# kchmck/p25rx

Measured on AMD Instinct MI355X. Metric: IQ Msamples/s through FM-demod+C4FM slice, higher is better.
Workload: dtype f32

## Files before the change

### p25rx_amd/csrc/p25fe_api.hip

```cpp
#include "p25fe_kernels.hip"

#include <hip/hip_ext.h>
#include <math.h>
#include <stdio.h>
#include <stdlib.h>
#include <string.h>

#include <algorithm>
#include <array>
#include <chrono>
#include <new>
#include <utility>
#include <string>
#include <vector>

#include "p25fe_jit.h"

using namespace p25k;

namespace {

constexpr size_t BBPAD = 256;
constexpr size_t SHARD_HALO = 2560;
static_assert(SHARD_HALO >= (size_t)(DEC * (PLPAD + CLK_L + 160) + TMAX) && 160 >= TMAX + TMAX - 1 && SHARD_HALO % 8 == 0, "shard halo");
// ... 221 lines not shown
    }
    void k1_events(bool ext_events, hipEvent_t* e0, hipEvent_t* e1)
    {
        *e0 = *e1 = nullptr;
        if (slot < 0 || !ext_events) return;
        *e0 = ev[(size_t)slot * 5 + 0]; *e1 = ev[(size_t)slot * 5 + 1];
        mask[(size_t)slot] |= 3u;
    }
};

constexpr size_t WIN_PARITY = 2, WIN_RING = 4;
struct WinSlot {
    hipEvent_t h2d_begin = nullptr, h2d_end = nullptr;
    hipEvent_t comp_begin = nullptr, comp_end = nullptr;
    hipEvent_t on_host = nullptr;
    std::array<hipEvent_t*, 5> all() { return {&h2d_begin, &h2d_end, &comp_begin, &comp_end, &on_host}; }
};
struct Windows {
    DevBuf buf[WIN_PARITY], dib[WIN_PARITY], res, anc;
    PinBuf stage[WIN_PARITY], out;
    hipStream_t cs = nullptr, os = nullptr;
    WinSlot slot[WIN_RING];
    WinSlot& of(size_t k) { return slot[k % WIN_RING]; }
    hipError_t ensure()
    {
        if (cs) return hipSuccess;
        hipError_t e = hipStreamCreateWithFlags(&cs, hipStreamNonBlocking);
        if (e == hipSuccess) e = hipStreamCreateWithFlags(&os, hipStreamNonBlocking);
        for (WinSlot& s : slot) for (hipEvent_t* x : s.all()) if (e == hipSuccess) e = hipEventCreate(x);
        return e;
    }
};

}

struct p25fe {
    p25fe_config_t cfg;
    int C = 1, n_cu = 256;
    Taps taps;
    int k1_p = 5;
    int variant = P25FE_VARIANT_BUILTIN;
    bool dflt = true;
    bool long_taps = false;
    int phase = P25FE_DECIM_PHASE;
    int n_avg = BOX;
    bool u8_lut_mode = false;
    float u8_scale = 0.0f, u8_offset = 0.0f;
    int track = 0;
    bool causal_ok = false;
    long look = 0;
    bool ext_events = true;
    int rx_cus = 0;
    int run_depth = 2;
    int sh_depth = MAX_LANES;

    int last_hip = 0;
    DevBuf d_taps;
    hipModule_t jit_mod = nullptr;
    hipFunction_t jit_fn[2][3] = {{nullptr, nullptr, nullptr}, {nullptr, nullptr, nullptr}};
    hipStream_t stream = nullptr, rx_stream = nullptr;
    const long* rs_idx = nullptr; size_t rs_n = 0, rs_stride = 0;
    Lane lanes[MAX_LANES];
    int cur = 0, lane_q[MAX_LANES - 1] = {1, 2, 3};
    int pl_lane = -1; size_t pl_blocks = 0;
    Lane& lane() { return lanes[cur]; }
    RxScratch& rx() { return lanes[cur].s; }
    const RxScratch& rx() const { return lanes[cur].s; }
    DevBuf power_partial, chunk_cnt, evrec, evnext, evoff;
    unsigned long long ev_seq = 0;
    PinBuf hin, hbb, hout;
    unsigned chunk_seq = 0;
    Windows win; StreamState state; Prof prof; ShardCtx sh;
};

struct PlanarGeo {
    size_t n_tiles, n_blocks;
    explicit PlanarGeo(size_t n_bb)
    {
        n_tiles = (n_bb + TS - 1) / TS;
        if (n_tiles == 0) n_tiles = 1;
        n_blocks = (size_t)TWORDS * n_tiles + 6;
    }
    size_t floats() const { return n_blocks * PL_BLK; }
    size_t words() const { return n_blocks * SPS; }
};

constexpr size_t MAX_RANGE_BB = (size_t)0x7ff00000u * 10u;
static inline bool position_refused(uint64_t pos) { return pos >= P25FE_MAX_POSITION; }

struct Resolved {
    Taps taps;
    bool long_taps;
    bool lut_affine;
    float u8_scale, u8_offset;
    bool dflt;
};

static inline bool finite_f(float v) { return v - v == 0.0f; }
static inline bool same_bits(float a, float b) { return memcmp(&a, &b, sizeof a) == 0; }

static bool lut_is_affine(const float* lut, float sc, float of)
{
    for (int b = 0; b < 256; ++b)
        if (!same_bits(lut[b], fmaf((float)b, sc, of))) return false;
    return true;
}
// ... 260 lines not shown
    try {
        h->state.reset((size_t)h->C);
    } catch (...) {
        return P25FE_ERR_NOMEM;
    }
    return P25FE_OK;
}

int p25fe_create(const p25fe_config_t* cfg, p25fe_t** out)
{
    if (!cfg || !out) return P25FE_ERR_ARG;
    *out = nullptr;
    if (cfg->abi_version != P25FE_ABI_VERSION || cfg->n_channels < 1 || cfg->n_channels > 65535 ) return P25FE_ERR_ARG;
    Resolved rs;
    if (int rrc = resolve_config(cfg, &rs)) return rrc;
    int ndev = 0;
    if (hipGetDeviceCount(&ndev) != hipSuccess || ndev <= 0 || cfg->device < 0 || cfg->device >= ndev)
        return P25FE_ERR_NO_DEVICE;
    if (hipSetDevice(cfg->device) != hipSuccess) return P25FE_ERR_NO_DEVICE;
    hipDeviceProp_t prop;
    if (hipGetDeviceProperties(&prop, cfg->device) != hipSuccess) return P25FE_ERR_NO_DEVICE;
    if (strncmp(prop.gcnArchName, "gfx950", 6) != 0) return P25FE_ERR_NO_DEVICE;

    p25fe_t* h = new (std::nothrow) p25fe;
    if (!h) return P25FE_ERR_NOMEM;
    h->cfg = *cfg;
    h->C = cfg->n_channels;
    h->track = cfg->symbol_clock & 0xff;
    h->causal_ok = (cfg->symbol_clock & P25FE_CLOCK_CAUSAL_OK) != 0;
    h->look = h->track ? CLK_L : 0;
    h->n_cu = prop.multiProcessorCount > 0 ? prop.multiProcessorCount : 256;
    h->taps = rs.taps;
    h->phase = cfg->decim_phase;
    h->n_avg = rs.taps.n_avg;
    h->long_taps = rs.long_taps;
    h->u8_lut_mode = !rs.lut_affine;
    h->u8_scale = rs.u8_scale; h->u8_offset = rs.u8_offset;
    h->variant = rs.dflt ? P25FE_VARIANT_BUILTIN : P25FE_VARIANT_GENERIC;
    h->dflt = rs.dflt;
    if (hipStreamCreateWithFlags(&h->stream, hipStreamNonBlocking) != hipSuccess) { p25fe_destroy(h); return P25FE_ERR_HIP; }
    hipError_t e = hipSuccess;
    {
        const char* pv = getenv("P25FE_K1_P");
        h->k1_p = (pv && atoi(pv) == 3) ? 3 : 5;
        const char* ee = getenv("P25FE_EXT_EVENTS");
        h->ext_events = !(ee && atoi(ee) == 0);
        const char* rc_ = getenv("P25FE_RX_CUS");
        h->rx_cus = rc_ ? atoi(rc_) : 0;
        const char* pd = getenv("P25FE_SHARD_PIPE_DEPTH");
        if (pd && atoi(pd) >= 2 && atoi(pd) <= MAX_LANES) h->sh_depth = atoi(pd);
        if (cfg->symbol_clock != P25FE_CLOCK_FIXED) h->run_depth = 3;
        const char* rd = getenv("P25FE_PIPE_DEPTH");
        if (rd && atoi(rd) >= 2 && atoi(rd) <= MAX_LANES) h->run_depth = atoi(rd);
    }
    if (e == hipSuccess) e = h->d_taps.ensure(sizeof(Taps));
    if (e == hipSuccess) e = hipMemcpy(h->d_taps.p, &h->taps, sizeof(Taps), hipMemcpyHostToDevice);
    if (e != hipSuccess) { p25fe_destroy(h); return P25FE_ERR_HIP; }
    {
        std::vector<char> code;
        std::string path;
        bool from_cache = false;
        int var = choose_variant(cfg, rs, &code, &path, &from_cache);
        if (var < 0) { p25fe_destroy(h); return var; }
        if (var == P25FE_VARIANT_SPECIALIZED) {
            bool ok = false;
            try {
                hipError_t me = hipModuleLoadData(&h->jit_mod, code.data());
                if (me != hipSuccess && from_cache) {
                    (void)hipGetLastError();
                    t_jit_log += "cached code object " + path + " did not load: recompiling\n";
                    const std::string store = p25jit::default_cache_dir();
                    if (path.compare(0, store.size() + 1, store + "/") == 0) (void)remove(path.c_str());
                    h->jit_mod = nullptr;
                    if (p25jit::get_code(jit_spec(rs), {}, true, store, false, code, path, t_jit_log)) me = hipModuleLoadData(&h->jit_mod, code.data());
                }
                ok = me == hipSuccess;
                for (int f = 0; f < 2 && ok; ++f)
                    for (int k = 0; k < 3 && ok; ++k)
                        ok = hipModuleGetFunction(&h->jit_fn[f][k], h->jit_mod, p25jit::KERNEL_NAMES[f][k]) == hipSuccess;
                if (!ok) { (void)hipGetLastError(); t_jit_log += "loading the specialised code object failed\n"; }
            } catch (...) {
                ok = false;
            }
            if (!ok) {
                if (h->jit_mod) { (void)hipModuleUnload(h->jit_mod); h->jit_mod = nullptr; }
                if (cfg->specialize >= P25FE_SPECIALIZE_REQUIRE) { p25fe_destroy(h); return P25FE_ERR_JIT; }
                var = rs.dflt ? P25FE_VARIANT_BUILTIN : P25FE_VARIANT_GENERIC;
                if (var == P25FE_VARIANT_GENERIC) fallback_notice();
            }
        }
        h->variant = var;
    }
    int rc = p25fe_reset(h);
    if (rc != P25FE_OK) { p25fe_destroy(h); return rc; }
    *out = h;
    return P25FE_OK;
}

void p25fe_destroy(p25fe_t* h)
{
    if (!h) return;
    (void)hipSetDevice(h->cfg.device);
    for (hipStream_t st : {h->stream, h->rx_stream, h->win.cs, h->win.os})
        if (st) { (void)hipStreamSynchronize(st); (void)hipStreamDestroy(st); }
    if (h->jit_mod) (void)hipModuleUnload(h->jit_mod);
    for (WinSlot& s : h->win.slot) for (hipEvent_t* e : s.all()) if (*e) (void)hipEventDestroy(*e);
    for (Lane& l : h->lanes)
        for (hipEvent_t e : {l.ev_k1, l.ev_rx}) if (e) (void)hipEventDestroy(e);
    for (auto& e : h->prof.ev) if (e) (void)hipEventDestroy(e);
    delete h;
}

}

enum K1Part { K1_ALL = 0, K1_MAIN = 1, K1_HEAD = 2 };
static int format_unusable(const p25fe_t* h, int fmt)
{
    const int v = format_variant_of(h->variant, h->dflt, h->cfg.specialize, fmt);
    return v < 0 ? v : P25FE_OK;
}
struct K1Launch {
    const void* src = nullptr;
    int fmt = P25FE_FMT_CF32;
    size_t ch_stride = 0, n_hist = 0, n = 0;
    uint64_t abs0 = 0;
    float* bb = nullptr; size_t bb_stride = 0;
    float* power_dbm = nullptr;
    bool planar = false;
    K1Part part = K1_ALL;
    hipEvent_t ev0 = nullptr, ev1 = nullptr;
    const ChunkRecvArgs* chunk = nullptr;
    long* head_end = nullptr;
    unsigned* done_flag = nullptr; unsigned done_seq = 0u;
    hipStream_t stream = nullptr;
};

struct K1Plan {
    bool empty;
    K1Args a;
    int fmt, variant; bool ct; int pk;
    long n_seg;
    long head_end;
    size_t lds;
};
static int k1_plan(const p25fe_t* h, const K1Launch& L, K1Plan* p)
{
    const int fmt = L.fmt;
    const int variant = format_variant_of(h->variant, h->dflt, h->cfg.specialize, fmt);
    if (variant < 0) return variant;
    if ((reinterpret_cast<uintptr_t>(L.src) & 15u) != 0) return P25FE_ERR_ARG;
    if (h->C > 1 && (L.ch_stride % fmt_stride_unit(fmt)) != 0) return P25FE_ERR_ARG;
    if (L.chunk && (!L.planar || L.part)) return P25FE_ERR_ARG;
    const bool pro = seg_prologue(fmt);
    const long m_begin = !L.planar ? 0 : (pro ? -(long)PLPAD - h->look : -(long)HIST_BB - h->look);
    const size_t n_out = p25fe_n_baseband_h(h, L.abs0, L.n);
    const long total = (long)n_out - m_begin;
    K1Args& a = p->a;
    a.m_begin = m_begin; a.n_out = (long)n_out; p->head_end = 0;
    p->empty = total <= 0;
    if (p->empty) return P25FE_OK;
    const int pk = (L.planar || h->long_taps || variant == P25FE_VARIANT_SPECIALIZED) ? 5 : h->k1_p;
    const int t1 = h->long_taps ? TMAX : T1;
    static const long subs_env = [] { const char* e = getenv("P25FE_SUBS"); return e ? atol(e) : 0L; }();
    long subs = subs_env > 0 ? subs_env : (fmt == P25FE_FMT_U8 ? 9 : (fmt == P25FE_FMT_S16 ? P25FE_K1_SUBS_S16 : 3));
    if (L.chunk) subs = 1;
    if (subs > 32768) subs = 32768;
    const bool ct = variant != P25FE_VARIANT_GENERIC;
    const int t2e = h->long_taps ? TMAX : T2;
    const int t3geo = ct ? h->n_avg : TMAX;
    SegGeo g{pro, WV * pk, (int)subs, seg_halo_for(h->n_avg, t2e), 0, m_begin, (long)n_out};
    const int nd = g.front(t3geo, t2e);
    const long o0 = (long)(((uint64_t)h->phase + 5 - L.abs0 % 5) % 5);
    if (L.part && subs > 1 && !L.chunk) g.set_lead(nd, o0, t1);
    const long n_seg = g.count(total);
    const long pl_shift = PLPAD + h->look;
    if (L.planar && !g.planar_ok(pl_shift)) return P25FE_ERR_ARG;
    if (L.planar && n_out > MAX_RANGE_BB) return P25FE_ERR_ARG;
    long seg_first = 0, seg_count = n_seg;
    if (L.part) {
        if (L.power_dbm) return P25FE_ERR_ARG;
        const long k_min = g.head_count(n_seg, nd, o0, t1);
        if (L.part == K1_MAIN) { seg_first = k_min; seg_count = n_seg - k_min; }
        else seg_count = k_min;
        p->head_end = g.start(k_min) - m_begin;
        p->empty = seg_count <= 0;
        if (p->empty) return P25FE_OK;
    }
    if (seg_count * (long)h->C > 0x7fffffffL) return P25FE_ERR_ARG;
    p->fmt = fmt; p->variant = variant; p->ct = ct; p->pk = pk; p->n_seg = n_seg;
    a.x = L.src; a.ch_stride = (long)L.ch_stride; a.n_hist = (long)L.n_hist; a.n_new = (long)L.n; a.o0 = (int)o0; a.n_ch = h->C;
    a.bb = L.bb; a.bb_stride = (long)L.bb_stride; a.power_partial = nullptr;
    a.subs_per_seg = g.subs_per_seg; a.seg_first = (int)seg_first; a.seg_count = (int)seg_count; a.lead_segs = g.lead_segs; a.seg_halo = g.segh;
    a.bbp = nullptr; a.bbp_ch_stride = 0; a.bits = nullptr; a.bits_ch_stride = 0; a.pl_shift = (int)pl_shift;
    a.done_flag = L.planar ? L.done_flag : nullptr; a.done_seq = L.done_seq;
    if (L.planar) {
        const PlanarGeo g(n_out);
        a.bbp = h->rx().pl_f.get(); a.bbp_ch_stride = (long)g.floats();
        a.bits = reinterpret_cast<uint8_t*>(h->rx().pl_bits.get()); a.bits_ch_stride = (long)(4 * g.words());
    }
    const bool lut = fmt == P25FE_FMT_U8 && (!ct || h->u8_lut_mode);
    p->lds = h->long_taps ? k1_lds_bytes<Geo<5, 1>>(ct, lut, t3geo) : (pk == 3 ? k1_lds_bytes<Geo<3>>(ct, lut, t3geo) : k1_lds_bytes<Geo<5>>(ct, lut, t3geo));
    static const size_t lds_pad_env = [] { const char* e = getenv("P25FE_K1_LDS_PAD"); return e ? (size_t)atol(e) : (size_t)0; }();
    p->lds += lds_pad_env;
    return P25FE_OK;
}

using K1Kernel = void (*)(K1Args, const Taps*);
using ChunkKernel = void (*)(K1Args, const Taps*, ChunkTail);
template <int FMT> static K1Kernel k1_kernel_of(bool ct, int pk, bool planar, bool long_taps)
{
    if (long_taps) return planar ? k_frontend<FMT, false, 5, OUT_PLANAR, 1> : k_frontend<FMT, false, 5, OUT_LINEAR, 1>;
    if (planar) return ct ? k_frontend<FMT, true, 5, OUT_PLANAR, 0> : k_frontend<FMT, false, 5, OUT_PLANAR, 0>;
    if (pk == 3) return ct ? k_frontend<FMT, true, 3, OUT_LINEAR, 0> : k_frontend<FMT, false, 3, OUT_LINEAR, 0>;
    return ct ? k_frontend<FMT, true, 5, OUT_LINEAR, 0> : k_frontend<FMT, false, 5, OUT_LINEAR, 0>;
}
template <int FMT> static ChunkKernel chunk_kernel_of(bool ct, bool long_taps)
{
    if (long_taps) return k_chunk<FMT, false, 1>;
    return ct ? k_chunk<FMT, true, 0> : k_chunk<FMT, false, 0>;
}
static K1Kernel k1_kernel_of(int fmt, bool ct, int pk, bool planar, bool long_taps)
{
    switch (fmt) {
    case P25FE_FMT_U8: return k1_kernel_of<P25FE_FMT_U8>(ct, pk, planar, long_taps);
    case P25FE_FMT_S16: return k1_kernel_of<P25FE_FMT_S16>(ct, pk, planar, long_taps);
    default: return k1_kernel_of<P25FE_FMT_CF32>(ct, pk, planar, long_taps);
    }
}
static ChunkKernel chunk_kernel_of(int fmt, bool ct, bool long_taps)
{
    switch (fmt) {
    case P25FE_FMT_U8: return chunk_kernel_of<P25FE_FMT_U8>(ct, long_taps);
    case P25FE_FMT_S16: return chunk_kernel_of<P25FE_FMT_S16>(ct, long_taps);
    default: return chunk_kernel_of<P25FE_FMT_CF32>(ct, long_taps);
    }
}

static int launch_k1(p25fe_t* h, const K1Launch& L)
{
    K1Plan p;
    if (int rc = k1_plan(h, L, &p)) return rc;
    if (L.head_end) *L.head_end = p.head_end;
    hipStream_t st = L.stream;
    if (p.empty) {
        if (L.power_dbm) HIPCHK(h, hipMemsetAsync(L.power_dbm, 0xff, sizeof(float) * (size_t)h->C, st));
        return P25FE_OK;
    }
    K1Args& a = p.a;
    if (L.power_dbm) {
        HIPCHK(h, h->power_partial.ensure(sizeof(float) * (size_t)h->C * (size_t)p.n_seg));
        a.power_partial = h->power_partial.as<float>();
    }
    ChunkTail tail;
    if (L.chunk) {
        if (!h->chunk_cnt.p) {
            HIPCHK(h, h->chunk_cnt.ensure(sizeof(unsigned) * (size_t)h->C));
            HIPCHK(h, hipMemsetAsync(h->chunk_cnt.p, 0, sizeof(unsigned) * (size_t)h->C, h->stream));
        }
        tail.r = *L.chunk; tail.counter = h->chunk_cnt.as<unsigned>(); tail.wg_per_ch = a.seg_count;
    }
    const Taps* dt = h->d_taps.as<Taps>();
    const dim3 grid((unsigned)a.seg_count, (unsigned)h->C);
    if (p.variant == P25FE_VARIANT_SPECIALIZED) {
        hipFunction_t f = h->jit_fn[p.fmt == P25FE_FMT_U8 ? 1 : 0][L.chunk ? 2 : (L.planar ? 1 : 0)];
        void* params[3] = {&a, &dt, &tail};
        if (L.ev0 || L.ev1)
            HIPCHK(h, hipExtModuleLaunchKernel(f, grid.x * WV, grid.y, 1, WV, 1, 1, p.lds, st, params, nullptr, L.ev0, L.ev1, 0));
        else
            HIPCHK(h, hipModuleLaunchKernel(f, grid.x, grid.y, 1, WV, 1, 1, (unsigned)p.lds, st, params, nullptr));
    } else if (L.chunk) {
        const ChunkKernel k = chunk_kernel_of(p.fmt, p.ct, h->long_taps);
        hipLaunchKernelGGL(k, grid, dim3(WV), p.lds, st, a, dt, tail);
    } else {
        const K1Kernel k = k1_kernel_of(p.fmt, p.ct, p.pk, L.planar, h->long_taps);
        launch_ev(k, grid, dim3(WV), p.lds, st, L.ev0, L.ev1, a, dt);
    }
    HIPCHK(h, hipGetLastError());
    if (L.power_dbm) {
        hipLaunchKernelGGL(k_power_finish, dim3((unsigned)h->C), dim3(256), 0, st, a.power_partial, (int)p.n_seg, a.n_out, L.power_dbm);
        HIPCHK(h, hipGetLastError());
    }
    return P25FE_OK;
}

static int ensure_slice_scratch(p25fe_t* h, size_t n_bb)
{
    const size_t C = (size_t)h->C;
    const PlanarGeo g(n_bb);
    const size_t nt = C * g.n_tiles, ng = C * (size_t)n_groups_of((int)g.n_tiles);
    RxScratch& s = h->rx();
    HIPCHK(h, s.pl_f.ensure(C * g.floats())); HIPCHK(h, s.pl_bits.ensure(C * g.words()));
    HIPCHK(h, s.evl.ensure(nt * EVCAP)); HIPCHK(h, s.evthr.ensure(nt * EVTHR_N * 3));
    HIPCHK(h, s.recs.ensure(nt)); HIPCHK(h, s.tsum.ensure(nt)); HIPCHK(h, s.outs.ensure(nt));
    HIPCHK(h, s.gagg.ensure(ng)); HIPCHK(h, s.gpre.ensure(ng));
    const unsigned* before = s.gtick.get();
    HIPCHK(h, s.gtick.ensure(ng + C));
    if (s.gtick.get() != before) HIPCHK(h, hipMemset(s.gtick.get(), 0, s.gtick.buf.cap));
    if (h->track || h->rs_n) {
        HIPCHK(h, s.gsum.ensure(nt)); HIPCHK(h, s.gouts.ensure(nt)); HIPCHK(h, s.evg.ensure(nt * EVCAP));
        HIPCHK(h, s.gsg.ensure(ng)); HIPCHK(h, s.gpg.ensure(ng));
    }
    h->pl_lane = h->cur; h->pl_blocks = g.n_blocks;
    return P25FE_OK;
}

struct RecvRange {
    size_t n_bb = 0;
    long abs_bb0 = 0;
    const p25fe_anchor_t* anchor_in = nullptr;
};
struct RecvDest {
    uint8_t* dibits = nullptr; size_t dibit_stride = 0;
    uint8_t* dibits2 = nullptr;
    int64_t* sync_pos = nullptr; uint64_t* sync_dibit = nullptr;
    size_t sync_stride = 0;
    p25fe_result_t* result = nullptr;
};
struct RecvCall {
    bool gen = false;
    bool reslice = false;
    RecvOpt opt;
    RecvRange range;
    RecvDest dest;
    bool detect = true;
    bool slice = true;
    bool wait_head = false;
    const ShardFix* fix = nullptr;
    hipEvent_t ev_done = nullptr;
// ... 1978 lines not shown
```

### p25rx_amd/csrc/p25fe_kernels.hip

```cpp
#ifndef __HIPCC_RTC__
#include <hip/hip_runtime.h>
#include <stdint.h>
#endif

#include "p25fe.h"
#include "p25fe_spec.h"

namespace p25k {

#ifdef P25FE_MEASURE
#include "p25fe_measure.inc"
#else
#define P25FE_M_LOAD_OFFSET(product_, cached_row_) (product_)
#define P25FE_M_ENTRY do { } while (0)
#define P25FE_M_LOCALS do { } while (0)
#define P25FE_M_ITEM do { } while (0)
#define P25FE_M_SUBTILE do { } while (0)
#define P25FE_M_EXIT do { } while (0)
#define K1_STAMP(i) do { } while (0)
#define K1_PIN2(a, b) do { } while (0)
#define P25FE_M_PIN_V2(arr_, n_) do { } while (0)
#define P25FE_M_PIN_F2(arr_, n_) do { } while (0)
#define P25FE_M_CUT_LOADS do { } while (0)
#define P25FE_M_CUT(stage_) do { } while (0)
#define P25FE_M_CUT_KEEP_F2(stage_, arr_, n_) do { } while (0)
#define P25FE_M_CUT_KEEP_F(stage_, arr_, n_) do { } while (0)
#define P25FE_M_KEEP1(a_) do { } while (0)
#define P25FE_M_KEEP2(a_, b_) do { } while (0)
#define P25FE_M_K6_STORES_ONLY do { } while (0)
#define P25FE_M_NO_BB_STORES false
#define P25FE_M_NO_SIGN_PLANES false
#define P25FE_M_NO_CH_FMA false
#define P25FE_M_NO_OUT_STAGE false
#define P25FE_M_DET_CUT_SCREEN do { } while (0)
#define P25FE_M_DET_NO_PEAK_TEST false
#define P25FE_M_PIPE_NOWAIT() false
#define P25FE_M_API_EXTRAS
#endif


template <int V> struct icst { static constexpr int value = V; };
template <bool B, class A, class C> struct cond { using type = A; };
template <class A, class C> struct cond<false, A, C> { using type = C; };

#ifdef P25FE_JIT
#define K1_CT_DECIM_TAPS P25FE_JIT_DECIM_TAPS
#define K1_CT_CHAN_TAPS P25FE_JIT_CHAN_TAPS
#define K1_CT_FM_GAIN P25FE_JIT_FM_GAIN
#define K1_CT_U8_SCALE P25FE_JIT_U8_SCALE
#define K1_CT_U8_OFFSET P25FE_JIT_U8_OFFSET
#define K1_CT_U8_LUT P25FE_JIT_U8_LUT
#define K1_CT_AVG_N P25FE_JIT_AVG_N
#define K1_CT_AVG_TAPS P25FE_JIT_AVG_TAPS
#define K1_CT_AVG_UNIFORM P25FE_JIT_AVG_UNIFORM
#else
#define K1_CT_DECIM_TAPS P25FE_DEFAULT_DECIM_TAPS
#define K1_CT_CHAN_TAPS P25FE_DEFAULT_CHAN_TAPS
#define K1_CT_FM_GAIN P25FE_FM_GAIN
#define K1_CT_U8_SCALE P25FE_U8_SCALE
#define K1_CT_U8_OFFSET P25FE_U8_OFFSET
#define K1_CT_U8_LUT 0
#define K1_CT_AVG_N P25FE_BOXCAR
#define K1_CT_AVG_TAPS P25FE_DEFAULT_AVG_TAPS
#define K1_CT_AVG_UNIFORM 1
#endif

constexpr int WV = 64;
constexpr int DEC = P25FE_DECIM;
constexpr int T1 = P25FE_T1;
constexpr int T2 = P25FE_T2;
constexpr int BOX = P25FE_BOXCAR;
constexpr int HALO_Y = BOX;
constexpr int HALO_D = HALO_Y + (T2 - 1);
constexpr int TMAX = P25FE_MAX_TAPS;
constexpr int AVG_DPP_MAX = 11;
constexpr int SEG_HALO = 80;
__host__ __device__ constexpr int seg_halo_for(int t3, int t2) { return t3 + t2 - 1 <= 80 ? 80 : 160; }
// ... 903 lines not shown
        return true;
    };
    if constexpr (PF == 1) {
        for (int it = 0; it < subs_this; ++it, dlo += SUB)
            if (!sub_tile(ld0)) break;
    } else {
        for (int it = 0; it < subs_this; it += 2) {
            if (!sub_tile(ld0)) break;
            dlo += SUB;
            if (it + 1 >= subs_this || !sub_tile(ld1)) break;
            dlo += SUB;
        }
    }
    flush_outputs();

    if (a.power_partial) {
#pragma unroll
        for (int d = 32; d > 0; d >>= 1) pw = pw + __shfl_down(pw, d, 64);
        if (tid == 0) a.power_partial[(size_t)ch * a.seg_count + seg_rel] = pw;
    }
    }
    if constexpr (OM == OUT_PLANAR) {
        if (a.done_flag) {
            asm volatile("s_waitcnt vmcnt(0)" ::: "memory");
            __builtin_amdgcn_fence(__ATOMIC_RELEASE, "agent");
            asm volatile("s_waitcnt vmcnt(0)" ::: "memory");
            unsigned ticket = 0u;
            if (tid == 0) ticket = __hip_atomic_fetch_add(a.done_flag + 1, 1u, __ATOMIC_RELAXED, __HIP_MEMORY_SCOPE_AGENT);
            ticket = (unsigned)__builtin_amdgcn_readfirstlane((int)ticket);
            if (ticket == gridDim.x * gridDim.y - 1u) {
                __builtin_amdgcn_fence(__ATOMIC_ACQUIRE, "agent");
                if (tid == 0) {
                    __hip_atomic_store(a.done_flag + 1, 0u, __ATOMIC_RELAXED, __HIP_MEMORY_SCOPE_AGENT);
                    __hip_atomic_store(a.done_flag, a.done_seq, __ATOMIC_RELEASE, __HIP_MEMORY_SCOPE_AGENT);
                }
            }
        }
    }
    P25FE_M_EXIT;
}

constexpr int k1_wps(int fmt, bool ct, int pk, int om)
{
    if (om == OUT_PLANAR)
        return fmt == P25FE_FMT_U8 ? (ct ? P25FE_K1_PLANAR_WPS_U8 : 2) : (fmt == P25FE_FMT_S16 ? (ct ? P25FE_K1_PLANAR_WPS_S16 : 2) : P25FE_K1_PLANAR_WPS);
    return (fmt == P25FE_FMT_U8 && !ct && pk <= 3) ? 3 : (pk <= 3 ? 4 : 2);
}
template <int FMT, bool CT, int PK, int OM = OUT_LINEAR, int TX = 0>
__global__ __launch_bounds__(WV, k1_wps(FMT, CT, PK, OM)) void k_frontend(K1Args a, const Taps* __restrict__ gtaps)
{
    frontend_body<FMT, CT, PK, OM, TX>(a, gtaps);
}

constexpr int PD = P25FE_PRE_DECIM;
constexpr int T0 = P25FE_T0;
#ifndef P25FE_K0_P
#define P25FE_K0_P 3
#endif
constexpr int K0_P = P25FE_K0_P;
constexpr int K0_SUB = WV * K0_P;
#ifndef P25FE_K0_SUBS
#define P25FE_K0_SUBS 2
#endif
#ifndef P25FE_K0_WPS
#define P25FE_K0_WPS 2
#endif
constexpr int K0_SUBS = P25FE_K0_SUBS;
constexpr int K0_HALO = T0 - PD;
constexpr int K0_NIN = PD * K0_SUB + K0_HALO;
constexpr int k0_row_pitch(int need) { return need + ((13 - need % 16) + 16) % 16; }
constexpr int K0_JP = k0_row_pitch(K0_NIN / PD + 2);
static_assert(K0_JP >= K0_NIN / PD + 2 && K0_JP % 16 == 13, "polyphase row pitch");
constexpr int HIST_PRE = K0_HALO + PD - 1;

struct K0Args {
    const float* x;
    long ch_stride;
    long n_hist, n_new;
    int o0;
    float* y;
    long y_stride;
    long n_out;
};

#ifndef P25FE_JIT
struct WideConv {
    float scale, offset;
    const float* lut;
};
constexpr int wide_log_spv(int fmt) { return fmt == P25FE_FMT_CF32 ? 1 : (fmt == P25FE_FMT_S16 ? 2 : 3); }
constexpr int wide_nv(int fmt, int nin) { return (nin + (1 << wide_log_spv(fmt)) + (WV << wide_log_spv(fmt)) - 1) / (WV << wide_log_spv(fmt)); }
template <int FMT, bool LUTM>
__device__ __forceinline__ float2 wide_sample(const uint4& v, int e, const WideConv& cv, const float* lut)
{
    static_assert(FMT == P25FE_FMT_CF32 || FMT == P25FE_FMT_S16 || FMT == P25FE_FMT_U8, "wideband formats");
    const unsigned w[4] = {v.x, v.y, v.z, v.w};
    if constexpr (FMT == P25FE_FMT_CF32) {
        return make_float2(__uint_as_float(w[2 * e]), __uint_as_float(w[2 * e + 1]));
    } else if constexpr (FMT == P25FE_FMT_S16) {
        return s16_to_c32(w[e]);
    } else {
        const unsigned pair = w[e >> 1] >> (16 * (e & 1));
        const unsigned bi = pair & 0xffu, bq = (pair >> 8) & 0xffu;
        if constexpr (LUTM) return make_float2(lut[bi], lut[bq]);
        else return make_float2(__builtin_fmaf((float)bi, cv.scale, cv.offset), __builtin_fmaf((float)bq, cv.scale, cv.offset));
    }
// ... 1020 lines not shown
```

### p25rx_amd/csrc/p25fe_measure.inc

```
#ifndef P25FE_MEASURE_INC
#define P25FE_MEASURE_INC

#ifndef P25FE_ABLATE
#define P25FE_ABLATE 99
#endif
#ifndef P25FE_EXP
#define P25FE_EXP 0
#endif

#if P25FE_ABLATE == 6 || defined(P25FE_ABLATE_CACHED)
#define P25FE_M_LOAD_OFFSET(product_, cached_row_) (cached_row_)
#else
#define P25FE_M_LOAD_OFFSET(product_, cached_row_) (product_)
#endif

#define P25FE_M_NO_BB_STORES ((P25FE_EXP & 8) != 0)
#define P25FE_M_NO_SIGN_PLANES ((P25FE_EXP & 1) != 0)
#define P25FE_M_NO_CH_FMA ((P25FE_EXP & 4) != 0)
#define P25FE_M_NO_OUT_STAGE (P25FE_ABLATE == 5)
#define P25FE_M_KEEP1(a_) asm volatile("" ::"v"(a_))
#define P25FE_M_KEEP2(a_, b_) asm volatile("" ::"v"(a_), "v"(b_))

#ifdef P25FE_K1_STAMP
constexpr int K1_STAMP_SLOTS = 8192;
// ... 20 lines not shown
#define P25FE_M_SUBTILE                                                               \
    do {                                                                              \
        asm volatile("s_memtime %0\n\ts_waitcnt lgkmcnt(0)" : "=s"(st_last)::"memory"); \
        if (st_first_sub) { st_pro += st_last - st_i0; st_first_sub = false; }        \
        ++st_n;                                                                       \
    } while (0)
#define P25FE_M_EXIT                                                                                                    \
    if (tid == 0) {                                                                                                     \
        unsigned long long st_t1, st_r1;                                                                                \
        asm volatile("s_memtime %0\n\ts_memrealtime %1\n\ts_waitcnt lgkmcnt(0)" : "=s"(st_t1), "=s"(st_r1)::"memory");  \
        unsigned long long* slot = g_k1_stamp[blockIdx.x % K1_STAMP_SLOTS];                                             \
        for (int i = 0; i < 7; ++i) atomicAdd(&slot[i], st_acc[i]);                                                     \
        atomicAdd(&slot[7], st_n);                                                                                      \
        atomicAdd(&slot[8], st_pro);                                    \
        atomicAdd(&slot[9], st_t1 - st_t0);                                                  \
        atomicAdd(&slot[10], st_r1 - st_r0);                                                \
        atomicAdd(&slot[11], 1ull);                                                                      \
        atomicAdd(&slot[12], st_items);                                                                  \
    }
#else
#define K1_STAMP(i) do { } while (0)
#define K1_PIN2(a, b) do { } while (0)
#define P25FE_M_PIN_V2(arr_, n_) do { } while (0)
#define P25FE_M_PIN_F2(arr_, n_) do { } while (0)
#define P25FE_M_ENTRY do { } while (0)
#define P25FE_M_LOCALS do { } while (0)
#define P25FE_M_ITEM do { } while (0)
#define P25FE_M_SUBTILE do { } while (0)
#define P25FE_M_EXIT do { } while (0)
#endif

#if P25FE_ABLATE <= 1
#if defined(P25FE_ABLATE_STORES)
#define P25FE_M_CUT_STORES_ out_rel = (int)(dlo - m_seg0);
#else
#define P25FE_M_CUT_STORES_
#endif
#if defined(P25FE_DRIFT)
#define P25FE_M_CUT_DRIFT_                                                                                   \
    {                                                                                                        \
        unsigned hsh = (unsigned)blockIdx.x * 2654435761u + (unsigned)(dlo & 0xffff) * 40503u;               \
        hsh ^= hsh >> 13;                                                                                    \
        const int units = P25FE_DRIFT + (int)(hsh % (unsigned)(P25FE_DRIFT_SPREAD + 1));                     \
        for (int u = 0; u < units; ++u) __builtin_amdgcn_s_sleep(1);                                         \
    }
#else
#define P25FE_M_CUT_DRIFT_
#endif
#define P25FE_M_CUT_LOADS do { P25FE_M_CUT_STORES_ P25FE_M_CUT_DRIFT_ return true; } while (0)
#else
#define P25FE_M_CUT_LOADS do { } while (0)
#endif
#define P25FE_M_CUT(stage_) do { if constexpr (P25FE_ABLATE <= (stage_)) return true; } while (0)
#define P25FE_M_CUT_KEEP_F2(stage_, arr_, n_)                                                                \
    do { if constexpr (P25FE_ABLATE <= (stage_)) {                                                           \
        _Pragma("unroll") for (int p_ = 0; p_ < (n_); ++p_) asm volatile("" ::"v"((arr_)[p_].x), "v"((arr_)[p_].y)); \
        return true; } } while (0)
#define P25FE_M_CUT_KEEP_F(stage_, arr_, n_)                                                                 \
    do { if constexpr (P25FE_ABLATE <= (stage_)) {                                                           \
        _Pragma("unroll") for (int p_ = 0; p_ < (n_); ++p_) asm volatile("" ::"v"((arr_)[p_]));              \
        return true; } } while (0)

#if defined(P25FE_ABLATE6)
#if P25FE_ABLATE6 == 2
#define P25FE_M_K6_STORES_ONLY                                                                               \
    {                                                                                                        \
        const float2 xv = lds_read_c(X + lane);                                                              \
        float4* const y4 = reinterpret_cast<float4*>(yb - (lane & 1));                                       \
        _Pragma("unroll 1") for (int c = 0; c < CZ_M; c += 2) {                                              \
            typedef float __attribute__((ext_vector_type(4))) f32x4;                                         \
            f32x4 ov; ov.x = xv.x + (float)c; ov.y = xv.y; ov.z = xv.x; ov.w = xv.y;                          \
            __builtin_nontemporal_store(ov, reinterpret_cast<f32x4*>(reinterpret_cast<float2*>(y4) + (size_t)(c + (lane & 1)) * a.y_stride)); \
        }                                                                                                    \
        return;                                                                                              \
    }
#else
#define P25FE_M_K6_STORES_ONLY                                                                               \
    {                                                                                                        \
        const float2 xv = lds_read_c(X + lane);                                                              \
        _Pragma("unroll 1") for (int c = 0; c < CZ_M; ++c) yb[(size_t)c * a.y_stride] = make_float2(xv.x + (float)c, xv.y); \
        return;                                                                                              \
    }
#endif
#else
#define P25FE_M_K6_STORES_ONLY do { } while (0)
#endif

#ifndef P25FE_ABLATE_DET
#define P25FE_ABLATE_DET 0
#endif
#define P25FE_M_DET_CUT_SCREEN                                                                               \
    do { if constexpr (P25FE_ABLATE_DET == 1) {                                                              \
        if (lane == 0) a.tsum[(size_t)ch * a.n_tiles + tile] = (hw[0] | hw[1] | hw[2] | hw[3]) == 0x12345u ? 1ull : 0ull; \
        return; } } while (0)
#define P25FE_M_DET_NO_PEAK_TEST (P25FE_ABLATE_DET == 2)

#ifdef P25FE_MEASURE_UNSAFE
#define P25FE_M_PIPE_NOWAIT() ([] { static const bool nowait = [] { const char* e = getenv("P25FE_PIPE_NOWAIT"); return e && atoi(e) != 0; }(); return nowait; }())
#else
#define P25FE_M_PIPE_NOWAIT() false
#endif
#ifdef P25FE_K1_STAMP
#define P25FE_M_API_EXTRAS                                                                                               \
    int p25fe_debug_k1_stamps(uint64_t out[16])                                                                          \
    {                                                                                                                    \
        std::vector<unsigned long long> z((size_t)p25k::K1_STAMP_SLOTS * 16, 0ull), v(z.size());                         \
// ... 12 lines not shown
```

Before: 537,800.

## Add producer/consumer paired-wave frontend kernel for planar CF32 path

Adds a new k_frontend_pair kernel with two waves per workgroup. One wave loads input and runs the decimating FIR into double-buffered LDS, while the other runs the channel filter, FM discriminator, averaging, and planar/bit-plane stores on the previous sub-block. Planning logic routes planar CF32 builtin launches to this kernel by default and reshapes the head part into a single-sub prologue launch. The aim is to overlap load/decimation with the downstream stages inside a CU. The cost is extra barriers, more LDS per workgroup, and more complex head/main segmentation that could change occupancy or correctness at boundaries.

Measured after the change: 569,100 (median of 6 runs). +5.8%, better.

```diff
diff --git a/p25rx_amd/csrc/p25fe_api.hip b/p25rx_amd/csrc/p25fe_api.hip
--- a/p25rx_amd/csrc/p25fe_api.hip
+++ b/p25rx_amd/csrc/p25fe_api.hip
@@ -297,6 +297,7 @@
     bool ext_events = true;
     int rx_cus = 0;
     int run_depth = 2;
+    bool k1_pair = true;
     int sh_depth = MAX_LANES;
 
     int last_hip = 0;
@@ -663,6 +664,8 @@
         if (cfg->symbol_clock != P25FE_CLOCK_FIXED) h->run_depth = 3;
         const char* rd = getenv("P25FE_PIPE_DEPTH");
         if (rd && atoi(rd) >= 2 && atoi(rd) <= MAX_LANES) h->run_depth = atoi(rd);
+        const char* kp = getenv("P25FE_K1_PAIR");
+        h->k1_pair = !(kp && atoi(kp) == 0);
     }
     if (e == hipSuccess) e = h->d_taps.ensure(sizeof(Taps));
     if (e == hipSuccess) e = hipMemcpy(h->d_taps.p, &h->taps, sizeof(Taps), hipMemcpyHostToDevice);
@@ -750,6 +753,7 @@
     bool empty;
     K1Args a;
     int fmt, variant; bool ct; int pk;
+    bool pair;
     long n_seg;
     long head_end;
     size_t lds;
@@ -762,36 +766,60 @@
     if ((reinterpret_cast<uintptr_t>(L.src) & 15u) != 0) return P25FE_ERR_ARG;
     if (h->C > 1 && (L.ch_stride % fmt_stride_unit(fmt)) != 0) return P25FE_ERR_ARG;
     if (L.chunk && (!L.planar || L.part)) return P25FE_ERR_ARG;
-    const bool pro = seg_prologue(fmt);
-    const long m_begin = !L.planar ? 0 : (pro ? -(long)PLPAD - h->look : -(long)HIST_BB - h->look);
-    const size_t n_out = p25fe_n_baseband_h(h, L.abs0, L.n);
-    const long total = (long)n_out - m_begin;
+    bool pro = seg_prologue(fmt);
+    long m_begin = !L.planar ? 0 : (pro ? -(long)PLPAD - h->look : -(long)HIST_BB - h->look);
+    const size_t n_out_range = p25fe_n_baseband_h(h, L.abs0, L.n);
+    long n_out = (long)n_out_range;
+    static const long subs_env = [] { const char* e = getenv("P25FE_SUBS"); return e ? atol(e) : 0L; }();
+    const long o0 = (long)(((uint64_t)h->phase + 5 - L.abs0 % 5) % 5);
+    K1Part part = L.part;
+    bool pair = false;
+    long pair_head = -1;
+    if (h->k1_pair && fmt == P25FE_FMT_CF32 && L.planar && variant == P25FE_VARIANT_BUILTIN && !h->long_taps && !L.chunk && !L.power_dbm) {
+        SegGeo gp{true, WV * 5, (int)(subs_env > 0 ? (subs_env > 32768 ? 32768 : subs_env) : 3), 0, 0, -(long)PLPAD - h->look, n_out};
+        const long tot = n_out - gp.m_begin;
+        const int ndp = gp.front(h->n_avg, T2);
+        if (L.part) gp.set_lead(ndp, o0, T1);
+        const long ns = tot > 0 ? gp.count(tot) : 0;
+        const long km = L.part ? gp.head_count(ns, ndp, o0, T1) : 0;
+        const long head_len = km >= ns ? tot : gp.start(km) - gp.m_begin;
+        if (tot - head_len >= gp.seg_len()) {
+            m_begin = gp.m_begin;
+            if (L.part == K1_HEAD) {
+                pair_head = head_len;
+                n_out = m_begin + head_len;
+                part = K1_ALL;
+            } else {
+                pair = true; pro = true;
+            }
+        }
+    }
+    const long total = n_out - m_begin;
     K1Args& a = p->a;
-    a.m_begin = m_begin; a.n_out = (long)n_out; p->head_end = 0;
+    a.m_begin = m_begin; a.n_out = n_out; p->pair = pair; p->head_end = pair_head > 0 ? pair_head : 0;
     p->empty = total <= 0;
     if (p->empty) return P25FE_OK;
     const int pk = (L.planar || h->long_taps || variant == P25FE_VARIANT_SPECIALIZED) ? 5 : h->k1_p;
     const int t1 = h->long_taps ? TMAX : T1;
-    static const long subs_env = [] { const char* e = getenv("P25FE_SUBS"); return e ? atol(e) : 0L; }();
     long subs = subs_env > 0 ? subs_env : (fmt == P25FE_FMT_U8 ? 9 : (fmt == P25FE_FMT_S16 ? P25FE_K1_SUBS_S16 : 3));
     if (L.chunk) subs = 1;
+    if (pair_head >= 0) subs = 1;
     if (subs > 32768) subs = 32768;
     const bool ct = variant != P25FE_VARIANT_GENERIC;
     const int t2e = h->long_taps ? TMAX : T2;
     const int t3geo = ct ? h->n_avg : TMAX;
-    SegGeo g{pro, WV * pk, (int)subs, seg_halo_for(h->n_avg, t2e), 0, m_begin, (long)n_out};
+    SegGeo g{pro, WV * pk, (int)subs, seg_halo_for(h->n_avg, t2e), 0, m_begin, n_out};
     const int nd = g.front(t3geo, t2e);
-    const long o0 = (long)(((uint64_t)h->phase + 5 - L.abs0 % 5) % 5);
-    if (L.part && subs > 1 && !L.chunk) g.set_lead(nd, o0, t1);
+    if (part && subs > 1 && !L.chunk) g.set_lead(nd, o0, t1);
     const long n_seg = g.count(total);
     const long pl_shift = PLPAD + h->look;
     if (L.planar && !g.planar_ok(pl_shift)) return P25FE_ERR_ARG;
-    if (L.planar && n_out > MAX_RANGE_BB) return P25FE_ERR_ARG;
+    if (L.planar && n_out_range > MAX_RANGE_BB) return P25FE_ERR_ARG;
     long seg_first = 0, seg_count = n_seg;
-    if (L.part) {
-        if (L.power_dbm) return P25FE_ERR_ARG;
+    if (L.part && L.power_dbm) return P25FE_ERR_ARG;
+    if (part) {
         const long k_min = g.head_count(n_seg, nd, o0, t1);
-        if (L.part == K1_MAIN) { seg_first = k_min; seg_count = n_seg - k_min; }
+        if (part == K1_MAIN) { seg_first = k_min; seg_count = n_seg - k_min; }
         else seg_count = k_min;
         p->head_end = g.start(k_min) - m_begin;
         p->empty = seg_count <= 0;
@@ -805,7 +833,7 @@
     a.bbp = nullptr; a.bbp_ch_stride = 0; a.bits = nullptr; a.bits_ch_stride = 0; a.pl_shift = (int)pl_shift;
     a.done_flag = L.planar ? L.done_flag : nullptr; a.done_seq = L.done_seq;
     if (L.planar) {
-        const PlanarGeo g(n_out);
+        const PlanarGeo g(n_out_range);
         a.bbp = h->rx().pl_f.get(); a.bbp_ch_stride = (long)g.floats();
         a.bits = reinterpret_cast<uint8_t*>(h->rx().pl_bits.get()); a.bits_ch_stride = (long)(4 * g.words());
     }
@@ -813,6 +841,7 @@
     p->lds = h->long_taps ? k1_lds_bytes<Geo<5, 1>>(ct, lut, t3geo) : (pk == 3 ? k1_lds_bytes<Geo<3>>(ct, lut, t3geo) : k1_lds_bytes<Geo<5>>(ct, lut, t3geo));
     static const size_t lds_pad_env = [] { const char* e = getenv("P25FE_K1_LDS_PAD"); return e ? (size_t)atol(e) : (size_t)0; }();
     p->lds += lds_pad_env;
+    if (pair) p->lds = PairGeo::LDS;
     return P25FE_OK;
 }
 
@@ -883,8 +912,8 @@
         const ChunkKernel k = chunk_kernel_of(p.fmt, p.ct, h->long_taps);
         hipLaunchKernelGGL(k, grid, dim3(WV), p.lds, st, a, dt, tail);
     } else {
-        const K1Kernel k = k1_kernel_of(p.fmt, p.ct, p.pk, L.planar, h->long_taps);
-        launch_ev(k, grid, dim3(WV), p.lds, st, L.ev0, L.ev1, a, dt);
+        const K1Kernel k = p.pair ? k_frontend_pair : k1_kernel_of(p.fmt, p.ct, p.pk, L.planar, h->long_taps);
+        launch_ev(k, grid, dim3(p.pair ? 2 * WV : WV), p.lds, st, L.ev0, L.ev1, a, dt);
     }
     HIPCHK(h, hipGetLastError());
     if (L.power_dbm) {
diff --git a/p25rx_amd/csrc/p25fe_kernels.hip b/p25rx_amd/csrc/p25fe_kernels.hip
--- a/p25rx_amd/csrc/p25fe_kernels.hip
+++ b/p25rx_amd/csrc/p25fe_kernels.hip
@@ -23,6 +23,8 @@
 #define P25FE_M_PIN_F2(arr_, n_) do { } while (0)
 #define P25FE_M_CUT_LOADS do { } while (0)
 #define P25FE_M_CUT(stage_) do { } while (0)
+#define P25FE_M_PAIR_PRODUCER_CUT do { } while (0)
+#define P25FE_M_PAIR_CONSUMER_CUT do { } while (0)
 #define P25FE_M_CUT_KEEP_F2(stage_, arr_, n_) do { } while (0)
 #define P25FE_M_CUT_KEEP_F(stage_, arr_, n_) do { } while (0)
 #define P25FE_M_KEEP1(a_) do { } while (0)
@@ -1032,6 +1034,257 @@
     frontend_body<FMT, CT, PK, OM, TX>(a, gtaps);
 }
 
+#ifndef P25FE_JIT
+struct PairGeo {
+    using G = Geo<5>;
+    static constexpr size_t XIN_B = sizeof(float2) * G::XIN_N;
+    static constexpr size_t DBUF_B = sizeof(float2) * G::D_N;
+    static constexpr size_t LDS = XIN_B + 2 * DBUF_B + sizeof(float) * G::SUB;
+    static_assert(XIN_B % 16 == 0 && DBUF_B % 16 == 0 && LDS <= 20480, "eight pair workgroups per CU");
+};
+__device__ __forceinline__ void pair_barrier()
+{
+    asm volatile("s_waitcnt lgkmcnt(0)\n\ts_barrier" ::: "memory");
+}
+__global__ __launch_bounds__(2 * WV, 4) void k_frontend_pair(K1Args a, const Taps* __restrict__)
+{
+    constexpr int FMT = P25FE_FMT_CF32;
+    using G = Geo<5>;
+    constexpr int P = 5, SUB = G::SUB, D_CARRY = G::D_CARRY;
+    constexpr int T3 = K1_CT_AVG_N, HY = T3;
+    constexpr int NBACK = (T3 - 1 + P - 1) / P;
+    static_assert(T3 >= 2 && T3 <= AVG_DPP_MAX && NBACK <= 3 && K1_CT_AVG_UNIFORM, "the build's own post-discriminator filter");
+    constexpr int ND = SegGeo{true}.front(HY, T2);
+    constexpr int PWIN = DEC * (ND - 1) + T1;
+    constexpr int NVP = (PWIN + 2 + 2 * WV - 1) / (2 * WV);
+    static_assert(ND <= WV && D_CARRY <= ND && 2 * ND <= SUB, "one prologue d per lane; PD_ fits OUT");
+    extern __shared__ __attribute__((aligned(16))) char smem[];
+    float2* const XIN = reinterpret_cast<float2*>(smem);
+    float2* const DB0 = XIN + G::XIN_N;
+    float2* const DB1 = DB0 + G::D_N;
+    float* const OUT = reinterpret_cast<float*>(DB1 + G::D_N);
+    float2* const PD_ = reinterpret_cast<float2*>(OUT);
+    const int tid = threadIdx.x & (WV - 1);
+    const int role = __builtin_amdgcn_readfirstlane((int)(threadIdx.x >> 6));
+    const int ch = (int)blockIdx.y;
+    const long seg = (long)blockIdx.x + a.seg_first;
+    const SegGeo sg = SegGeo{true, SUB, a.subs_per_seg, 0}.range(a.lead_segs, a.m_begin, a.n_out);
+    const long m_seg0 = sg.start(seg);
+    const long m_seg1 = sg.end(seg);
+    const int n_sub = m_seg0 < a.n_out ? (int)((m_seg1 - m_seg0 + SUB - 1) / SUB) : 0;
+    const float fm_gain = K1_CT_FM_GAIN;
+    if (n_sub > 0) {
+    if (role == 0) {
+        const char* xb = reinterpret_cast<const char*>(a.x) + (size_t)ch * a.ch_stride * fmt_bps(FMT);
+        Loader<FMT, P> ld0;
+        Loader<FMT, P, 0, NVP> lp;
+        const long i_last = (long)a.o0 + DEC * (m_seg1 - 1);
+        const long pfirst = K1_FIRST_INPUT(m_seg0 - ND, a.o0, T1);
+        ld0.init(xb, pfirst, a.n_hist, a.n_new, i_last);
+        lp.rs = ld0.rs; lp.base_idx = ld0.base_idx;
+        lp.load_first(pfirst, tid);
+        lp.store(XIN, pfirst, a.n_hist, a.n_new, tid);
+        lp.fixup(XIN, pfirst, a.n_hist, a.n_new, tid);
+        ld0.load_first(K1_FIRST_INPUT(m_seg0, a.o0, T1), tid);
+        phase_sync();
+        {
+            v2f dacc = v2f{0.f, 0.f};
+            const float2* w = XIN + (int)(pfirst & 1) + DEC * tid;
+            lds_walk<T1, true>(w, [&](auto jc, v2f sv) {
+                constexpr int j = decltype(jc)::value;
+                dacc = cfma(K1_CT_DECIM_TAPS[T1 - 1 - j], sv, dacc);
+            });
+            if (tid < ND) PD_[tid] = make_float2(dacc.x, dacc.y);
+            if (tid >= ND - D_CARRY && tid < ND) DB0[tid - (ND - D_CARRY)] = make_float2(dacc.x, dacc.y);
+        }
+        pair_barrier();
+        long dlo = m_seg0;
+        for (int t = 0; t < n_sub; ++t, dlo += SUB) {
+            float2* const Dc = (t & 1) ? DB1 : DB0;
+            const float2* const Dp = (t & 1) ? DB0 : DB1;
+            const long first = K1_FIRST_INPUT(dlo, a.o0, T1);
+            const int xsh = (int)(first & 1);
+#if P25FE_K1_TURNAROUND_PRIO
+            __builtin_amdgcn_s_setprio(P25FE_K1_TURNAROUND_PRIO);
+#endif
+            ld0.store(XIN, first, a.n_hist, a.n_new, tid);
+            {
+                int tidf = tid;
+                asm volatile("" : "+v"(tidf));
+                ld0.fixup(XIN, first, a.n_hist, a.n_new, tidf);
+            }
+            phase_sync();
+            ld0.load(first + (long)DEC * SUB, tid);
+#if P25FE_K1_TURNAROUND_PRIO
+            __builtin_amdgcn_s_setprio(0);
+#endif
+            P25FE_M_PAIR_PRODUCER_CUT;
+            if (t > 0 && tid < D_CARRY) Dc[tid] = lds_read_c(Dp + SUB + tid);
+            const float2* w = XIN + xsh + (DEC * P) * tid;
+            v2f acc[P];
+#pragma unroll
+            for (int p = 0; p < P; ++p) acc[p] = v2f{0.f, 0.f};
+            lds_walk<DEC * (P - 1) + T1, true>(w, [&](auto jc, v2f s) {
+                constexpr int j = decltype(jc)::value;
+#pragma unroll
+                for (int p = 0; p < P; ++p) {
+                    const int k = DEC * p + (T1 - 1) - j;
+                    if (k >= 0 && k < T1) acc[p] = cfma(K1_CT_DECIM_TAPS[k], s, acc[p]);
+                }
+            });
+            phase_sync();
+#pragma unroll
+            for (int p = 0; p < P; ++p) Dc[D_CARRY + P * tid + p] = make_float2(acc[p].x, acc[p].y);
+            pair_barrier();
+        }
+    } else {
+        float2 y_carry;
+        float f_carry[NBACK][P];
+        pair_barrier();
+        {
+            v2f yv = v2f{0.f, 0.f};
+            if (tid < HY) {
+                const float2* w = PD_ + (ND - HY) - (T2 - 1) + tid;
+                lds_walk<T2, true>(w, [&](auto jc, v2f sv) {
+                    constexpr int j = decltype(jc)::value;
+                    yv = cfma(K1_CT_CHAN_TAPS[T2 - 1 - j], sv, yv);
+                });
+            }
+            float2 yp;
+            yp.x = wave_shr1(yv.x, 0.f);
+            yp.y = wave_shr1(yv.y, 0.f);
+            const float fmv = fm_discriminate(make_float2(yv.x, yv.y), yp, fm_gain);
+            y_carry.x = lane_bcast<HY - 1>(yv.x);
+            y_carry.y = lane_bcast<HY - 1>(yv.y);
+            static_for<0, NBACK>([&](auto bc) {
+                constexpr int b = decltype(bc)::value;
+                static_for<0, P>([&](auto pc) {
+                    constexpr int p = decltype(pc)::value;
+                    constexpr int l = HY - (b + 1) * P + p;
+                    if constexpr (l >= 1) f_carry[b][p] = lane_bcast<l>(fmv);
+                    else f_carry[b][p] = 0.f;
+                });
+            });
+            phase_sync();
+        }
+        float outv[P];
+#pragma unroll
+        for (int q = 0; q < P; ++q) outv[q] = 0.f;
+        int out_rel = -2 * SUB;
+        const int seg_n = (int)(m_seg1 - m_seg0);
+        const int pl_sym = tid & 31, pl_h5 = (tid >> 5) * 5;
+        const int i_seg = (int)((m_seg0 + a.pl_shift) / SPS_);
+        float* const bbp_ch = a.bbp + (size_t)ch * a.bbp_ch_stride;
+        unsigned* const bits_ch = reinterpret_cast<unsigned*>(a.bits + (size_t)ch * a.bits_ch_stride);
+        unsigned bitsv = 0u;
+        auto flush_outputs = [&]() {
+            const int blk = (i_seg >> 5) + out_rel / SUB;
+            float* const row = bbp_ch + (size_t)blk * PL_BLK + pl_sym + 32 * pl_h5;
+#pragma unroll
+            for (int q = 0; q < P; ++q) {
+                const int r = out_rel + SPS_ * pl_sym + pl_h5 + q;
+#if P25FE_K1_NT_STORES
+                if (r >= 0 && r < seg_n) __builtin_nontemporal_store(outv[q], row + 32 * q);
+#else
+                if (r >= 0 && r < seg_n) row[32 * q] = outv[q];
+#endif
+            }
+            if (tid < SPS_ && out_rel >= 0 && out_rel < seg_n) bits_ch[(size_t)blk * SPS_ + tid] = bitsv;
+        };
+        for (int t = 0; t < n_sub; ++t) {
+            const float2* const Dc = (t & 1) ? DB1 : DB0;
+            flush_outputs();
+            pair_barrier();
+            P25FE_M_PAIR_CONSUMER_CUT;
+            float2 y[P];
+            {
+                const float2* w = Dc + (D_CARRY - (T2 - 1)) + P * tid;
+                v2f yv[P];
+#pragma unroll
+                for (int p = 0; p < P; ++p) yv[p] = v2f{0.f, 0.f};
+                lds_walk<(P - 1) + T2, true>(w, [&](auto jc, v2f s) {
+                    constexpr int j = decltype(jc)::value;
+#pragma unroll
+                    for (int p = 0; p < P; ++p) {
+                        const int k = p + (T2 - 1) - j;
+                        if (k >= 0 && k < T2) yv[p] = cfma(K1_CT_CHAN_TAPS[k], s, yv[p]);
+                    }
+                });
+#pragma unroll
+                for (int p = 0; p < P; ++p) y[p] = make_float2(yv[p].x, yv[p].y);
+            }
+            float f[P];
+            {
+                float2 yprev;
+                yprev.x = wave_shr1(y[P - 1].x, y_carry.x);
+                yprev.y = wave_shr1(y[P - 1].y, y_carry.y);
+                f[0] = fm_discriminate(y[0], yprev, fm_gain);
+#pragma unroll
+                for (int p = 1; p < P; ++p) f[p] = fm_discriminate(y[p], y[p - 1], fm_gain);
+                y_carry.x = lane_bcast<WV - 1>(y[P - 1].x);
+                y_carry.y = lane_bcast<WV - 1>(y[P - 1].y);
+            }
+            {
+                float prevf[NBACK][P];
+#pragma unroll
+                for (int p = 0; p < P; ++p) prevf[0][p] = wave_shr1(f[p], f_carry[0][p]);
+#pragma unroll
+                for (int b = 1; b < NBACK; ++b)
+#pragma unroll
+                    for (int p = 0; p < P; ++p) prevf[b][p] = wave_shr1(prevf[b - 1][p], f_carry[b][p]);
+                auto fm_back = [&](int p, int j) -> float {
+                    const int q = p - j;
+                    if (q >= 0) return f[q];
+                    const int b = (-q + P - 1) / P;
+                    return prevf[b - 1][q + b * P];
+                };
+#pragma unroll
+                for (int p = 0; p < P; ++p) {
+                    float acc = f[p];
+#pragma unroll
+                    for (int j = 1; j < T3; ++j) acc = acc + fm_back(p, j);
+                    acc = acc * K1_CT_AVG_TAPS[0];
+                    OUT[P * tid + p] = acc;
+                }
+#pragma unroll
+                for (int p = 0; p < P; ++p) {
+                    if constexpr (NBACK >= 3) f_carry[2][p] = lane_bcast<WV - 3>(f[p]);
+                    if constexpr (NBACK >= 2) f_carry[1][p] = lane_bcast<WV - 2>(f[p]);
+                    f_carry[0][p] = lane_bcast<WV - 1>(f[p]);
+                }
+            }
+            phase_sync();
+            unsigned long long sgn[5];
+#pragma unroll
+            for (int q = 0; q < P; ++q) {
+                outv[q] = OUT[SPS_ * pl_sym + pl_h5 + q];
+                sgn[q] = __builtin_amdgcn_ballot_w64(__float_as_int(outv[q]) < 0);
+            }
+            bitsv = lanes_from_ballots(sgn);
+            out_rel = t * SUB;
+            phase_sync();
+        }
+        flush_outputs();
+    }
+    }
+    if (role == 1 && a.done_flag) {
+        asm volatile("s_waitcnt vmcnt(0)" ::: "memory");
+        __builtin_amdgcn_fence(__ATOMIC_RELEASE, "agent");
+        asm volatile("s_waitcnt vmcnt(0)" ::: "memory");
+        unsigned ticket = 0u;
+        if (tid == 0) ticket = __hip_atomic_fetch_add(a.done_flag + 1, 1u, __ATOMIC_RELAXED, __HIP_MEMORY_SCOPE_AGENT);
+        ticket = (unsigned)__builtin_amdgcn_readfirstlane((int)ticket);
+        if (ticket == gridDim.x * gridDim.y - 1u) {
+            __builtin_amdgcn_fence(__ATOMIC_ACQUIRE, "agent");
+            if (tid == 0) {
+                __hip_atomic_store(a.done_flag + 1, 0u, __ATOMIC_RELAXED, __HIP_MEMORY_SCOPE_AGENT);
+                __hip_atomic_store(a.done_flag, a.done_seq, __ATOMIC_RELEASE, __HIP_MEMORY_SCOPE_AGENT);
+            }
+        }
+    }
+}
+#endif
+
 constexpr int PD = P25FE_PRE_DECIM;
 constexpr int T0 = P25FE_T0;
 #ifndef P25FE_K0_P
diff --git a/p25rx_amd/csrc/p25fe_measure.inc b/p25rx_amd/csrc/p25fe_measure.inc
--- a/p25rx_amd/csrc/p25fe_measure.inc
+++ b/p25rx_amd/csrc/p25fe_measure.inc
@@ -96,6 +96,17 @@
 #define P25FE_M_CUT_LOADS do { } while (0)
 #endif
 #define P25FE_M_CUT(stage_) do { if constexpr (P25FE_ABLATE <= (stage_)) return true; } while (0)
+#if P25FE_ABLATE <= 1
+#define P25FE_M_PAIR_PRODUCER_CUT { pair_barrier(); continue; }
+#if defined(P25FE_ABLATE_STORES)
+#define P25FE_M_PAIR_CONSUMER_CUT { out_rel = t * SUB; continue; }
+#else
+#define P25FE_M_PAIR_CONSUMER_CUT { continue; }
+#endif
+#else
+#define P25FE_M_PAIR_PRODUCER_CUT do { } while (0)
+#define P25FE_M_PAIR_CONSUMER_CUT do { } while (0)
+#endif
 #define P25FE_M_CUT_KEEP_F2(stage_, arr_, n_)                                                                \
     do { if constexpr (P25FE_ABLATE <= (stage_)) {                                                           \
         _Pragma("unroll") for (int p_ = 0; p_ < (n_); ++p_) asm volatile("" ::"v"((arr_)[p_].x), "v"((arr_)[p_].y)); \
```
